# smly/RiichiEnv

Hardware: AMD Instinct MI355X
Metric: env.step()/s (whole node) at 65 536 parallel 4p games; bit-exact MJAI parity (higher is better)
Workload: dtype u8

## Files before the change

riichienv_amd/csrc/rmj_step4.hip.h:

```cpp
namespace RMJ_NS {

#define R4_LIST 16
#define R4_ACT_CAP (KSANMA ? 2 * R4_LIST : R4_LIST)
#define R4_RE_DRAW 1u
#define R4_RE_RESTART 2u
#define R4_RE_PUB 3u
#define R4_RE_YAKU_CLAIMS 4u
#define R4_RE_YAKU_TSUMO 5u
#define R4_RE_WIN_TSUMO 6u
#define R4_RE_WIN_RON 7u
#define R4_RET_ROUND 0x100u
#define STEP_F_ROWS_SHIFT 20
__device__ __forceinline__ uint32_t r4_rows(uint32_t flags) {
    const uint32_t c = (flags >> STEP_F_ROWS_SHIFT) & 3u;
    return c == 0u ? 4u : c;
}
#ifdef RMJ_CUTS
#define R4M(id) do { if (rmj::g_cut == (id)) asm volatile("s_endpgm" ::: "memory"); } while (0)
#define R4BAIL(q, id) do { (q).bail = true; if ((q).r == 0) atomicAdd(&rmj::g_bail_reason[id], 1u); } while (0)
#else
#define R4M(id) do {} while (0)
#ifdef RMJ_CENSUS
#define R4BAIL(q, id) do { (q).bail = true; (q).why = (id); } while (0)
#elif defined(RMJ_TL4)
// ... 253 lines not shown
            const bool ok = live && r4_word_ok(w + (1u << sh3), s, tot);
            W |= (uint64_t)(rballot(ok, rb) & 0x1FFu) << (9 * s);
        }
    }
    const int pairs = __popc(h.a & O9_2 & ~(h.a << 1)) + __popc(h.b & O9_2 & ~(h.b << 1)) + __popc(h.c & O9_2 & ~(h.c << 1)) +
                      __popc(h.d & O7_2 & ~(h.d << 1));
    const uint32_t pres_d = (h.d | (h.d >> 1) | (h.d >> 2)) & O7_1;
    const int kinds = __popc(pres_d) + ((h.a & 7u) != 0u) + ((h.a >> 24) != 0u) + ((h.b & 7u) != 0u) + ((h.b >> 24) != 0u) +
                      ((h.c & 7u) != 0u) + ((h.c >> 24) != 0u);
    if (__ballot(pairs >= 6 || kinds >= 12)) {
        if (pairs >= 6) {
            const uint32_t odd_a = h.a & O9_1, odd_b = h.b & O9_1, odd_c = h.c & O9_1, odd_d = h.d & O7_1;
            const uint32_t four = (h.a & O9_4) | (h.b & O9_4) | (h.c & O9_4) | (h.d & O7_4);
            const int n_odd = __popc(odd_a) + __popc(odd_b) + __popc(odd_c) + __popc(odd_d);
            const int n_two = __popc(h.a & O9_2) + __popc(h.b & O9_2) + __popc(h.c & O9_2) + __popc(h.d & O7_2);
            if (four == 0u && n_odd == 1 && n_two == 6) {
                const int t = odd_a ? (__ffs((int)odd_a) - 1) / 3 : (odd_b ? 9 + (__ffs((int)odd_b) - 1) / 3 : (odd_c ? 18 + (__ffs((int)odd_c) - 1) / 3 : 27 + (__ffs((int)odd_d) - 1) / 3));
                if (ph_cnt(h, t) == 1) W |= 1ull << t;
            }
        }
        if (kinds >= 12) {
            const int t = r < 6 ? (r >> 1) * 9 + (r & 1) * 8 : 27 + (r - 6);
            bool kw = false;
            if (r < 13 && ph_cnt(h, t) < 4) {
                PH x = h;
                ph_add(x, t);
                kw = is_kokushi(x);
            }
            const uint32_t kb = rballot(kw, rb);
            uint64_t kmask = 0ull;
#pragma unroll
            for (int i = 0; i < 13; i++) {
                const int ti = i < 6 ? (i >> 1) * 9 + (i & 1) * 8 : 27 + (i - 6);
                kmask |= (uint64_t)((kb >> i) & 1u) << ti;
            }
            W |= kmask;
        }
    }
    return W;
}

template <bool RICH>
__device__ __forceinline__ void r4_fill_waits13(R4& q, PState* P, int n) {
    uint64_t W = 0ull;
    const R4Shape sp = r4_shape_sorted(q, P, n);
    const int iso = sp.iso, yaochu = sp.yaochu;
    int lb = iso >= 6 ? 4 : (iso == 5 ? 3 : (iso == 4 ? 2 : 0));
    const int len3 = n / 3;
    if (len3 == 4) {
        const int koku = 12 - yaochu;
        lb = koku < lb ? koku : lb;
        if (lb > 2) {
            const int chi = 6 - sp.pairs + (sp.kinds < 7 ? 7 - sp.kinds : 0);
            lb = chi < lb ? chi : lb;
        }
    }
    int sh = lb;
    if (lb < 2) {
        bool far = iso >= 2 && yaochu < 12;
        if (q.gf && !far && !(len3 == 4 && (sp.pairs >= 6 || yaochu >= 12))) {
            const uint32_t gr = r4_group_residues(sp.start, sp.S, n, q.r, q.rb);
            far = gr != 0x01u && gr != 0x20u;
        }
        if (far) {
            sh = 1;
        } else {
            PH h13 = {0, 0, 0, 0};
            {
                uint32_t a = 0, b = 0, c = 0, d = 0;
                if (q.r < n) {
                    const int t = P->hand[q.r] >> 2, su = t_suit(t);
                    const uint32_t one = 1u << (3 * (t - 9 * su));
                    a = su == 0 ? one : 0u; b = su == 1 ? one : 0u; c = su == 2 ? one : 0u; d = su == 3 ? one : 0u;
                }
                a = row_sum16(a); b = row_sum16(b); c = row_sum16(c); d = row_sum16(d);
                const int l15 = q.rb + 15;
                h13.a = (uint32_t)rbc((int)a, l15); h13.b = (uint32_t)rbc((int)b, l15); h13.c = (uint32_t)rbc((int)c, l15); h13.d = (uint32_t)rbc((int)d, l15);
            }
            sh = r4_shanten(q, h13, len3);
            if (sh <= 0) {
                if (!RICH) { R4BAIL(q, 2); return; }
                W = r4_waits_probe(h13.a, h13.b, h13.c, h13.d);
                sh = 0;
            }
        }
    }
    if (q.r == 0) {
        P->waits13 = W;
        P->sh13 = (uint8_t)sh;
        P->flags |= PF_WAITS_VALID;
    }
    wave_sync();
}

template <bool RICH>
__device__ __forceinline__ void r4_fill_waits13_h(R4& q, PState* P, const PH& h13) {
    uint64_t W = 0ull;
    const uint32_t T9 = 1u | (1u << 24);
    const int yaochu = __popc((h13.a | (h13.a >> 1) | (h13.a >> 2)) & T9) + __popc((h13.b | (h13.b >> 1) | (h13.b >> 2)) & T9) +
                       __popc((h13.c | (h13.c >> 1) | (h13.c >> 2)) & T9) + __popc((h13.d | (h13.d >> 1) | (h13.d >> 2)) & O7_1);
    const int iso = r4_isolated(h13);
    int lb = iso >= 6 ? 4 : (iso == 5 ? 3 : (iso == 4 ? 2 : 0));
    const int len3 = ph_total(h13) / 3;
    if (len3 == 4) {
        const int koku = 12 - yaochu;
        lb = koku < lb ? koku : lb;
        if (lb > 2) {
            const int chi = sh_chiitoi(h13, false);
            lb = chi < lb ? chi : lb;
        }
    }
    int sh = lb;
    if (lb < 2) {
        if (iso >= 2 && yaochu < 12) {
            sh = 1;
        } else {
            sh = r4_shanten(q, h13, len3);
            if (sh <= 0) {
                if (!RICH) { R4BAIL(q, 2); return; }
                W = r4_waits_probe(h13.a, h13.b, h13.c, h13.d);
                sh = 0;
            }
        }
    }
    if (q.r == 0) {
        P->waits13 = W;
        P->sh13 = (uint8_t)sh;
        P->flags |= PF_WAITS_VALID;
    }
    wave_sync();
}

__device__ __forceinline__ void r4_accept_riichi(R4& q) {
    GState* G = q.G;
    const int p = G->riichi_pending;
    if (p != 0xFF) {
        q.dirty |= 1u << p;
        if (q.r == 0) {
            G->p[p].score -= 1000;
            G->p[p].score_delta -= 1000;
            G->riichi_sticks += 1;
            G->p[p].flags |= PF_RIICHI_DECLARED | PF_IPPATSU;
            G->riichi_pending = 0xFF;
        }
        wave_sync();
        r4_emit_simple(q, RMJ_EV_REACH_ACCEPTED, (uint32_t)p, 0);
    }
}
__device__ __forceinline__ void r4_check_abortive(R4& q) {
    GState* G = q.G;
    const int p = (q.r >> 2) & 3, m = q.r & 3;
    const PState& P = G->p[p];
    const bool seat_lane = m == 0;
    const int nm = P.n_melds;
    const uint32_t turns_ok = rballot(seat_lane && P.n_discards == 1, q.rb);
    const uint32_t has_melds = rballot(seat_lane && nm != 0, q.rb);
    const uint32_t riichi = rballot(seat_lane && (P.flags & PF_RIICHI_DECLARED), q.rb);
    const uint32_t kan = rballot(m < nm && P.meld_type[m] >= RMJ_MELD_DAIMINKAN, q.rb);
    const uint32_t all_seats = 0x1111u;
    if (!KSANMA && turns_ok == all_seats && has_melds == 0u) {
        const int first = G->p[0].discards[0] >> 2;
        if (first >= 27 && first <= 30) {
            const uint32_t same = rballot(seat_lane && (P.discards[0] >> 2) == first, q.rb);
            if (same == all_seats) R4BAIL(q, 4);
        }
    }
    if (__popc(kan) == 4) {
        const int owner = (__ffs((int)kan) - 1) >> 2;
        if (kan & ~(0xFu << (4 * owner))) R4BAIL(q, 5);
    }
    if (!KSANMA && riichi == all_seats) R4BAIL(q, 6);
}
__device__ __forceinline__ void r4_deal_next(R4& q, int pf) {
    GState* G = q.G;
    const int drawable = G->drawable_count;
    if (drawable == 0) {
        if (q.pause_ok) q.rend = 1u ;
        else { R4BAIL(q, 7); q.cont = 1; }
        return;
    }
    const int live_end = G->live_end;
    const int pid = G->current_player;
    PState* P = &G->p[pid];
    const int hl = P->hand_len;
    if (live_end > G->rinshan_count) {
        q.dirty |= 1u << pid;
        if (q.r == 0) {
            G->is_rinshan = 0;
            G->live_end = (uint8_t)(live_end - 1);
            G->drawable_count = (uint8_t)(drawable - 1);
            if (hl < 14) { P->hand[hl] = (uint8_t)pf; P->hand_len = (uint8_t)(hl + 1); }
            G->drawn_tile = (uint8_t)pf;
            G->needs_tsumo = 0;
            G->phase = RMJ_WAIT_ACT;
            G->active_mask = (uint8_t)(1u << pid);
            P->n_forbidden = 0;
        }
        wave_sync();
        r4_emit_simple(q, RMJ_EV_TSUMO, (uint32_t)pid, (uint32_t)pf);
    } else if (q.r == 0) {
        G->is_rinshan = 0;
    }
}
__device__ __forceinline__ void r4_turn_end(R4& q, int pf) {
    GState* G = q.G;
    r4_accept_riichi(q);
    if (q.tend == 1) r4_check_abortive(q);
    if (q.bail) return;
    const uint32_t tc = G->turn_count + 1u;
    const int pid = G->current_player;
    if (q.r == 0) {
        G->turn_count = tc;
        G->current_player = (uint8_t)(pid + 1 == KNP ? 0 : pid + 1);
    }
    wave_sync();
    r4_deal_next(q, pf);
    if (q.bail) return;
    if (q.r == 0 && tc >= (uint32_t)KNP) G->is_first_turn = 0;
    wave_sync();
}

__device__ __forceinline__ int r4_tile_id(int t34) {
    return KSANMA ? (t34 == 0 ? 0 : (t34 == 8 ? 1 : t34 - 7)) : t34;
}
__device__ __forceinline__ void r4_put(R4& q, int seat, int pos, uint64_t a, int id) {
    if (pos < R4_ACT_CAP) (&q.T->lst[q.row][seat][0])[pos] = a | ((uint64_t)(uint32_t)id << 56);
}

template <bool LOOP>
__device__ __forceinline__ int r4_wall_tile(const R4& q, int idx) {
    const uint8_t* Wg = q.E->wall + (size_t)q.g * RMJ_WALL_STRIDE;
    if (LOOP) {
        const uint32_t w = __hip_atomic_load(reinterpret_cast<const uint32_t*>(Wg) + (idx >> 2), __ATOMIC_RELAXED, __HIP_MEMORY_SCOPE_AGENT);
        return (int)((w >> (8 * (idx & 3))) & 0xFFu);
    }
    return Wg[idx];
}
template <bool LOOP>
__device__ __forceinline__ void r4_flush_kan_dora(R4& q, int extra) {
    GState* G = q.G;
    int pk = (int)G->pending_kan_dora + extra;
    while (__ballot(pk > 0)) {
        if (pk > 0) {
            pk -= 1;
            const int count = G->n_dora;
            const int widx = KSANMA ? 8 + 2 * count : 4 + 2 * count;
            const bool flip = count < 5 && (KSANMA || widx < (int)G->live_end);
            const int t = flip ? r4_wall_tile<LOOP>(q, widx) : 0;
            if (q.r == 0) {
                G->pending_kan_dora = (uint8_t)(pk >= extra ? pk - extra : 0);
                if (flip) { G->dora[count] = (uint8_t)t; G->n_dora = (uint8_t)(count + 1); }
            }
            wave_sync();
            if (flip) r4_emit_simple(q, RMJ_EV_DORA, 0u, (uint32_t)t);
        }
    }
}
template <bool LOOP>
__device__ __forceinline__ void r4_kan_draw(R4& q, int pid, PState* P, bool ankan, uint32_t ev_w0, uint32_t ev_cons, uint32_t ev_n) {
    GState* G = q.G;
    const int r = q.r;
    if (G->drawable_count == 0) { R4BAIL(q, 29); return; }
    if (r < 4) G->p[r].flags &= ~PF_IPPATSU;
    const int rc = G->rinshan_count;
    const int t = r4_wall_tile<LOOP>(q, rc);
    if (r == 0) {
        G->is_first_turn = 0;
        G->rinshan_count = (uint8_t)(rc + 1);
        G->drawable_count -= 1;
        const int h2 = P->hand_len;
        if (h2 < 14) { P->hand[h2] = (uint8_t)t; P->hand_len = (uint8_t)(h2 + 1); }
        G->drawn_tile = (uint8_t)t;
        G->is_rinshan = 1;
    }
    wave_sync();
    if (ev_w0) r4_emit(q, ev_w0, ev_cons, (ev_n << 4) & 0xFFu);
    r4_flush_kan_dora<LOOP>(q, ankan ? 1 : 0);
    if (!ankan && r == 0) G->pending_kan_dora += 1;
    wave_sync();
    r4_emit_simple(q, RMJ_EV_TSUMO, (uint32_t)pid, (uint32_t)t);
    if (r == 0) {
        G->phase = RMJ_WAIT_ACT;
        G->active_mask = (uint8_t)(1u << pid);
    }
    wave_sync();
}
template <bool SETTLE>
__device__ __forceinline__ E4Out r4_seat_eval(uint32_t on, uint32_t seat, uint32_t tile, uint32_t cf, uint32_t honba, bool use_ura, const uint8_t* Wg) {
    const int lane = threadIdx.x & 63, row = lane >> 4, r = lane & 15, rb = lane & 48;
    const GState* G = &g_q4.st[row];
    const PState* P = &G->p[seat & 3u];
    const bool act = on != 0u;
    const int hl = act ? (int)P->hand_len : 0, nm = act ? (int)P->n_melds : 0;
    const int tid = r < hl ? (int)P->hand[r] : 0;
    uint32_t ca = 0, cb = 0, cc = 0, cd = 0;
    if (r < hl) {
        const int t = tid >> 2, su = t_suit(t);
        const uint32_t one = 1u << (3 * (t - 9 * su));
        ca = su == 0 ? one : 0u; cb = su == 1 ? one : 0u; cc = su == 2 ? one : 0u; cd = su == 3 ? one : 0u;
    }
    PH h;
    h.a = e4_rsum(ca, rb); h.b = e4_rsum(cb, rb); h.c = e4_rsum(cc, rb); h.d = e4_rsum(cd, rb);
    int aka = __popc(e4_ballot(r < hl && is_aka(tid), rb));
    uint32_t ma_ = 0, mb_ = 0, mc_ = 0, md_ = 0;
    E4Meld mp;
    {
        const bool mv = r < nm;
        const int m = r & 3;
        const uint32_t type = P->meld_type[m];
        const int nt = type >= RMJ_MELD_DAIMINKAN ? 4 : 3;
        const uint32_t t0 = P->meld_tiles[m][0], t1 = P->meld_tiles[m][1], t2 = P->meld_tiles[m][2], t3 = P->meld_tiles[m][3];
        if (mv) {
#pragma unroll
            for (int k = 0; k < 4; k++) {
                const int t = (int)(k == 0 ? t0 : (k == 1 ? t1 : (k == 2 ? t2 : t3))) >> 2;
                if (k < nt) {
                    const int su = t_suit(t);
                    const uint32_t one = 1u << (3 * (t - 9 * su));
                    ma_ += su == 0 ? one : 0u; mb_ += su == 1 ? one : 0u; mc_ += su == 2 ? one : 0u; md_ += su == 3 ? one : 0u;
                }
            }
        }
        mp = e4_meld_lane(mv, type, nt, t0, t1, t2, t3, (int)((type == RMJ_MELD_CHI ? min(t0, min(t1, t2)) : t0) >> 2), type != RMJ_MELD_CHI,
                          type != RMJ_MELD_ANKAN);
// ... 135 lines not shown
    const PState& S4 = G->p[r & 3];
    const bool other = r < KNP && r != pid;
    const uint32_t qfl = S4.flags;
    const bool holds13 = other && (S4.hand_len + 3 * S4.n_melds == 13);
    const uint64_t W = holds13 ? S4.waits13 : 0ull;
    const uint32_t riichi_m = rballot(r < 4 && (qfl & PF_RIICHI_DECLARED), rb) & 0xFu;
    uint32_t ron_m = 0u;
    if (__ballot(((W >> tt) & 1ull) != 0ull)) {
        const uint64_t dtm = S4.discard_type_mask;
        const bool in_discards = (dtm >> tt) & 1ull;
        const bool in_missed = (qfl & PF_MISSED_DOUJUN) || ((qfl & PF_RIICHI_DECLARED) && (qfl & PF_MISSED_RIICHI));
        const bool furiten = (W & dtm) != 0ull || (qfl & (PF_MISSED_RIICHI | PF_MISSED_DOUJUN));
        ron_m = rballot(other && !in_discards && !in_missed && !furiten && ((W >> tt) & 1ull), rb) & 0xFu;
    }
    if (ron_m && !RICH) { R4BAIL(q, 9); return; }
    if (RICH && (ron_m & ~riichi_m)) {
        if (!RESUME) {
            if (q.pause_ok) q.rend = R4_RE_YAKU_CLAIMS; else R4BAIL(q, 9);
            return;
        }
        const uint32_t ok_m = (ron_m & riichi_m) | (q.yk & ron_m & ~riichi_m), miss_m = (q.yk >> 4) & ron_m & ~riichi_m;
        if (r < 4 && ((miss_m >> r) & 1u)) G->p[r].flags |= PF_MISSED_DOUJUN;
        q.dirty |= miss_m;
        ron_m = ok_m;
        wave_sync();
    }
    w_mine = r < 4 ? W : 0ull;
    const bool can_call = G->drawable_count > 0;
    const bool kuikae = (q.E->rule_bits & RMJ_RULE_KUIKAE_FORBIDDEN) != 0;
    R4M(52);
    int nl0 = (RICH && (ron_m & 1u)) ? 1 : 0, nl1 = (RICH && (ron_m & 2u)) ? 1 : 0, nl2 = (RICH && (ron_m & 4u)) ? 1 : 0, nl3 = (RICH && (ron_m & 8u)) ? 1 : 0;
    auto nl_get = [&](int i) { return i == 0 ? nl0 : (i == 1 ? nl1 : (i == 2 ? nl2 : nl3)); };
    auto nl_set = [&](int i, int v) {
        nl0 = i == 0 ? v : nl0; nl1 = i == 1 ? v : nl1; nl2 = i == 2 ? v : nl2; nl3 = i == 3 ? v : nl3;
    };
#pragma unroll
    for (int k = 1; k < KNP; k++) {
        const int i = pid + k >= KNP ? pid + k - KNP : pid + k;
        const PState* Q = &G->p[i];
        const int hl = Q->hand_len;
        const int ht = r < hl ? (int)Q->hand[r] : 0xFF;
        const uint32_t sm = can_call ? rballot(r < hl && (ht >> 2) == tt, rb) : 0u;
        const int count = __popc(sm);
        if (count < 2 || ((riichi_m >> i) & 1u)) continue;
        const int i0 = __ffs((int)sm) - 1;
        const uint32_t m1 = sm & (sm - 1u);
        const int i1 = __ffs((int)m1) - 1;
        const int i2 = count >= 3 ? __ffs((int)(m1 & (m1 - 1u))) - 1 : 0;
        const uint32_t h0 = (uint32_t)rbc(ht, rb + i0), h1 = (uint32_t)rbc(ht, rb + i1), h2 = (uint32_t)rbc(ht, rb + i2);
        int n = nl_get(i);
        if (r == 0) {
            if (hl >= 3 && (kuikae ? (hl - count) > 0 : (hl - 2) > 0)) {
                r4_put(q, i, n, mk_action(RMJ_PON, tile, 2, h0, h1), KSANMA ? 28 : 41);
                if (count >= 3) {
                    r4_put(q, i, n + 1, mk_action(RMJ_PON, tile, 2, h0, h2), KSANMA ? 28 : 41);
                    r4_put(q, i, n + 2, mk_action(RMJ_PON, tile, 2, h1, h2), KSANMA ? 28 : 41);
                }
            }
        }
        if (hl >= 3 && (kuikae ? (hl - count) > 0 : (hl - 2) > 0)) n += count >= 3 ? 3 : 1;
        if (count >= 3) {
            if (r == 0) r4_put(q, i, n, mk_action(RMJ_DAIMINKAN, tile, 3, h0, h1, h2), (KSANMA ? 29 : 42) + r4_tile_id(tt));
            n += 1;
        }
        nl_set(i, n);
    }
    R4M(53);
    if (!KSANMA && can_call && tt < 27) {
        const int i = (pid + 1) & 3;
        const PState* Q = &G->p[i];
        const int hl = Q->hand_len;
        if (!((riichi_m >> i) & 1u) && hl >= 3) {
            const int ht = r < hl ? (int)Q->hand[r] : 0xFF;
            const int hty = ht >> 2;
            const int r9 = tt % 9;
            const uint32_t m_m2 = rballot(r < hl && hty == tt - 2, rb), m_m1 = rballot(r < hl && hty == tt - 1, rb);
            const uint32_t m_p1 = rballot(r < hl && hty == tt + 1, rb), m_p2 = rballot(r < hl && hty == tt + 2, rb);
            if ((m_m2 && m_m1) || (m_m1 && m_p1) || (m_p1 && m_p2)) {
                const uint32_t m_0 = rballot(r < hl && hty == tt, rb);
                const uint32_t m_p3 = rballot(r < hl && hty == tt + 3, rb), m_m3 = rballot(r < hl && hty == tt - 3, rb);
                const int a = (r >> 2) & 3, b = r & 3;
                int n = nl_get(i);
#pragma unroll
                for (int k = 0; k < 3; k++) {
                    const bool pat_ok = k == 0 ? (r9 >= 2) : (k == 1 ? (r9 >= 1 && r9 <= 7) : (r9 <= 6));
                    const uint32_t ma = k == 0 ? m_m2 : (k == 1 ? m_m1 : m_p1);
                    const uint32_t mbb = k == 0 ? m_m1 : (k == 1 ? m_p1 : m_p2);
                    if (!__ballot(pat_ok && ma != 0u && mbb != 0u)) continue;
                    int forb = __popc(m_0);
                    if (k == 2 && r9 <= 5) forb += __popc(m_p3);
                    if (k == 0 && r9 >= 3) forb += __popc(m_m3);
                    const bool kk_ok = kuikae ? (hl - 2 - forb) > 0 : (hl - 2) > 0;
                    const bool valid = pat_ok && a < __popc(ma) && b < __popc(mbb) && kk_ok;
                    uint32_t x = ma, y = mbb;
                    for (int s = 0; s < a; s++) x &= x - 1u;
                    for (int s = 0; s < b; s++) y &= y - 1u;
                    const int ia = valid ? __ffs((int)x) - 1 : 0, ib = valid ? __ffs((int)y) - 1 : 0;
                    const uint32_t ta = (uint32_t)rbc(ht, rb + ia), tb = (uint32_t)rbc(ht, rb + ib);
                    const uint32_t vb = rballot(valid, rb);
                    if (valid) r4_put(q, i, n + __popc(vb & ((1u << r) - 1u)), mk_action(RMJ_CHI, tile, 2, ta, tb), 40 - k);
                    n += __popc(vb);
                }
                nl_set(i, n);
            }
        }
    }
    R4M(54);
    int n_me = r < 4 ? nl_get(r) : 0;
    if (RICH && ron_m) {
        if (r < 4 && ((ron_m >> r) & 1u)) q.T->lst[q.row][r][0] = mk_action(RMJ_RON, tile, 0) | ((uint64_t)(KSANMA ? 56 : 79) << 56);
        if (r == 0) G->ron_offer_mask = (uint8_t)ron_m;
    }
    if (rballot(r < 4 && n_me + 1 > R4_LIST, rb)) { R4BAIL(q, 10); return; }
    if (r < 4) {
        G->stale_n[r] = (uint8_t)(n_me > 62 ? 62 : n_me);
        if (n_me > 0) {
            q.T->lst[q.row][r][n_me] = mk_action(RMJ_PASS, RMJ_TILE_NONE, 0) | ((uint64_t)(KSANMA ? 58 : 81) << 56);
            n_me += 1;
        }
    }
    nl_mine = r < 4 ? n_me : 0;
    const uint32_t claim_active = rballot(r < 4 && n_me > 0, rb) & 0xFu;
    wave_sync();
    R4M(55);
    if (claim_active) {
        if (r == 0) {
            G->phase = RMJ_WAIT_RESPONSE;
            G->active_mask = (uint8_t)claim_active;
        }
        wave_sync();
    } else {
        q.tend = 1;
    }
}

__device__ __forceinline__ uint32_t r4_tenpai_keep(const R4& q, const PState* P, const PH& full, int hl);
template <bool RICH>
__device__ __forceinline__ void r4_gen_act_legal(R4& q, int& nl_mine) {
    GState* G = q.G;
    const int r = q.r, rb = q.rb;
    const int pid = G->current_player;
    PState* P = &G->p[pid];
    const int hl = P->hand_len, nmelds = P->n_melds;
    const uint32_t pflags = P->flags;
    const bool r_decl = pflags & PF_RIICHI_DECLARED, r_stage = pflags & PF_RIICHI_STAGE;
    const int drawn_tile = G->drawn_tile;
    const bool drawn = drawn_tile != 0xFF;
    const int drawable = G->drawable_count;
    if (hl + 3 * nmelds == 13 || (!RICH && r_stage)) { R4BAIL(q, 11); return; }
    const int ht = r < hl ? (int)P->hand[r] : 0xFF;
    const int hty = ht >> 2;
    int n = 0;
    int d_idx = -1;
    if (drawn && !r_stage) {
        const uint32_t b = rballot(r < hl && ht == drawn_tile, rb);
        const int idx = b ? 31 - __clz((int)b) : -1;
        d_idx = idx;
        const int same_type = __popc(rballot(r < hl && hty == (drawn_tile >> 2), rb));
        if (!(idx >= 0 && same_type <= 4 && (hl - 1) + 3 * nmelds == 13)) { R4BAIL(q, 12); return; }
        if (!(pflags & PF_WAITS_VALID)) {
            const int nx = __builtin_amdgcn_update_dpp(0xFFFF, ht, 0x101 , 0xf, 0xf, false);
            if (idx != hl - 1 || rballot(r < hl - 2 && ht > nx, rb)) r4_fill_waits13_h<RICH>(q, P, r4_hist(q, P, idx));
            else r4_fill_waits13<RICH>(q, P, hl - 1);
            if (q.bail) return;
        }
        if ((P->waits13 >> (drawn_tile >> 2)) & 1ull) {
            const bool concealed = rballot(r < nmelds && P->meld_type[r & 3] != RMJ_MELD_ANKAN, rb) == 0u;
            if (!RICH) { R4BAIL(q, 13); return; }
            bool offer = concealed;
            if (!concealed) {
                if (q.yk_mode == R4_RE_YAKU_TSUMO) offer = (q.yk & 1u) != 0u;
                else if (q.pause_ok) { q.rend = R4_RE_YAKU_TSUMO; return; }
                else { R4BAIL(q, 13); return; }
            }
            if (offer) {
                if (r == 0) r4_put(q, pid, n, mk_action(RMJ_TSUMO, drawn_tile, 0), KSANMA ? 56 : 79);
                n += 1;
            }
        }
    }
    R4M(60);
    const int nforb = P->n_forbidden;
    const bool forb = (nforb > 0 && (P->forbidden[0] >> 2) == hty) || (nforb > 1 && (P->forbidden[1] >> 2) == hty);
    const PH full = r4_hist(q, P, -1);
    if (r_decl) {
        if (drawn) {
            if (r == 0) r4_put(q, pid, n, mk_action(RMJ_DISCARD, drawn_tile, 0), r4_tile_id(drawn_tile >> 2));
            n += 1;
        }
    } else {
        const bool all_closed = rballot(r < nmelds && P->meld_type[r & 3] != RMJ_MELD_ANKAN, rb) == 0u;
        const bool riichi_pre = !r_stage && P->score >= 1000 && (KSANMA ? drawable > 0 : drawable >= 4) && all_closed;
        bool need_tp = r_stage;
        if (riichi_pre) {
            const int sh13 = (drawn && (P->flags & PF_WAITS_VALID)) ? (int)P->sh13 : -1;
            if (sh13 < 2) {
                auto yaochu_kinds = [&]() {
                    const uint32_t T9 = 1u | (1u << 24);
                    return __popc((full.a | (full.a >> 1) | (full.a >> 2)) & T9) + __popc((full.b | (full.b >> 1) | (full.b >> 2)) & T9) +
                           __popc((full.c | (full.c >> 1) | (full.c >> 2)) & T9) + __popc((full.d | (full.d >> 1) | (full.d >> 2)) & O7_1);
                };
                bool may;
                const int nx14 = __builtin_amdgcn_update_dpp(0xFFFF, ht, 0x101 , 0xf, 0xf, false);
                if (q.gf && d_idx == hl - 1 && rballot(r < hl - 2 && ht > nx14, rb) == 0u) {
                    const bool in = r < hl;
                    const int k = in ? r4_key(hty) : 1000;
                    const int kd = rbc(k, rb + hl - 1);
                    const int m = __popc(rballot(r < hl - 1 && k <= kd, rb));
                    const int ks = __builtin_amdgcn_update_dpp(-1000, k, 0x111 , 0xf, 0xf, false);
                    const int k14 = !in ? 1000 : (r < m ? k : (r == m ? kd : ks));
                    const int kp = __builtin_amdgcn_update_dpp(-1000, k14, 0x111 , 0xf, 0xf, false);
                    const bool start = in && k14 - kp > 2;
                    const uint32_t S = rballot(start, rb);
                    const uint32_t gr = r4_group_residues(start, S, hl, r, rb);
                    may = gr == 0x10u || gr == 0x02u || gr == 0x21u;
                    if (!may && hl == 14) {
                        const int kn = __builtin_amdgcn_update_dpp(1000, k14, 0x101 , 0xf, 0xf, false);
                        may = __popc(rballot(in && k14 != kp && k14 == kn, rb)) >= 6 || (__popc(S) >= 12 && yaochu_kinds() >= 12);
                    }
                } else {
                    may = !(r4_isolated(full) >= 3 && yaochu_kinds() < 12);
                }
                if (may) {
                    if (r4_shanten(q, full, hl / 3) <= 0) {
                        if (!RICH) { R4BAIL(q, 14); return; }
                        need_tp = true;
                    }
                }
            }
        }
        uint32_t tp = 0u;
        if (r_stage && G->tp_seat == pid && G->tp_step == G->step_count) {
            tp = G->tp_mask;
            need_tp = false;
        }
        if (RICH && __ballot(need_tp)) {
            if (need_tp) {
                tp = r4_tenpai_keep(q, P, full, hl);
                if (r == 0 && !r_stage) { G->tp_seat = (uint8_t)pid; G->tp_mask = (uint16_t)tp; G->tp_step = G->step_count + 1u; }
            }
        }
        const bool ok = r < hl && !forb && (!r_stage || ((tp >> r) & 1u));
        const uint32_t vb = rballot(ok, rb);
        if (ok) r4_put(q, pid, n + __popc(vb & ((1u << r) - 1u)), mk_action(RMJ_DISCARD, ht, 0), r4_tile_id(hty));
        n += __popc(vb);
        if (riichi_pre && tp != 0u) {
            if (r == 0) r4_put(q, pid, n, mk_action(RMJ_RIICHI, RMJ_TILE_NONE, 0), KSANMA ? 27 : 37);
            n += 1;
        }
    }
    R4M(61);
    if (drawable > 0 && drawn) {
        if (!r_decl && !r_stage) {
            const bool any4 = (((full.a | full.b | full.c) & O9_4) | (full.d & O7_4)) != 0u;
            if (any4) {
                const int next_t = __builtin_amdgcn_update_dpp(0xFFFF, ht, 0x101 , 0xf, 0xf, false);
                if (rballot(r < hl - 2 && ht > next_t, rb)) { R4BAIL(q, 15); return; }
                const int prev_ty = __builtin_amdgcn_update_dpp(-1, hty, 0x111 , 0xf, 0xf, false);
                const bool is4 = r < hl - 1 && hty != prev_ty && ph_cnt(full, hty) == 4;
                const uint32_t ab = rballot(is4, rb);
                if (is4) {
                    const uint32_t lo = (uint32_t)hty * 4u;
                    r4_put(q, pid, n + __popc(ab & ((1u << r) - 1u)), mk_action(RMJ_ANKAN, lo, 4, lo, lo + 1, lo + 2, lo + 3),
                           (KSANMA ? 29 : 42) + r4_tile_id(hty));
                }
                n += __popc(ab);
            }
            const uint32_t pon_lane = rballot(r < nmelds && P->meld_type[r & 3] == RMJ_MELD_PON, rb);
            if (pon_lane) {
                for (int m = 0; m < nmelds; m++) {
                    if (P->meld_type[m] != RMJ_MELD_PON) continue;
                    const int target = P->meld_tiles[m][0] >> 2;
                    const bool hit = r < hl && hty == target;
                    const uint32_t kb = rballot(hit, rb);
                    if (hit)
                        r4_put(q, pid, n + __popc(kb & ((1u << r) - 1u)),
                               mk_kakan(ht, P->meld_tiles[m][0], P->meld_tiles[m][1], P->meld_tiles[m][2]),
                               (KSANMA ? 29 : 42) + r4_tile_id(target));
                    n += __popc(kb);
                }
            }
        } else if (r_decl) {
            if (ph_cnt(full, drawn_tile >> 2) == 4) { R4BAIL(q, 16); return; }
        }
    }
    if (G->is_first_turn && !r_stage && (G->p[0].n_melds | G->p[1].n_melds | G->p[2].n_melds | G->p[3].n_melds) == 0) {
        const bool term = r < hl && is_terminal_tile136(ht);
        const uint32_t lo = row_or16(term && hty < 32 ? 1u << hty : 0u), hi = row_or16(term && hty >= 32 ? 1u << (hty - 32) : 0u);
        const int kinds = __popc((uint32_t)rbc((int)lo, rb + 15)) + __popc((uint32_t)rbc((int)hi, rb + 15));
        if (kinds >= 9) {
            if (r == 0) r4_put(q, pid, n, mk_action(RMJ_KYUSHU, RMJ_TILE_NONE, 0), KSANMA ? 57 : 80);
            n += 1;
        }
    }
    if (KSANMA && drawn && drawable > 0) {
        const bool hit = r < hl && hty == 30;
        const uint32_t kb = rballot(hit, rb);
        if (hit) r4_put(q, pid, n + __popc(kb & ((1u << r) - 1u)), mk_action(RMJ_KITA, ht, 0), 59);
        n += __popc(kb);
    }
    if (n > R4_ACT_CAP) { R4BAIL(q, 17); return; }
    nl_mine = r == pid ? n : 0;
    wave_sync();
}

__device__ __forceinline__ void r4_emit_now(R4& q, bool on, uint32_t w) {
    if (q.E->skip_log) return;
    const uint32_t evc = q.G->ev_count;
    wave_sync();
    if (on) {
        uint32_t* dst = reinterpret_cast<uint32_t*>(q.E->events + (size_t)q.g * (q.E->ring_mask + 1u) + (evc & q.E->ring_mask));
        if (q.r < 8) dst[q.r] = q.r == 7 ? ((w & 0x00FFFFFFu) | ((uint32_t)KNP << 24)) : w;
        if (q.r == 0) q.G->ev_count = evc + 1u;
    }
    wave_sync();
}
#ifdef RMJ_RE_PROF
#define RE_MARK(k) do { const unsigned long long t__ = __builtin_amdgcn_s_memrealtime(); if (lane == 0) atomicAdd(&rmj::g_re_prof[k], t__ - re_t); re_t = t__; } while (0)
#define RE_ROWS(md) do { if ((threadIdx.x & 15u) == 0u) atomicAdd(&rmj::g_re_prof[8 + ((md) & 15u)], 1ull); } while (0)
#define RE_STAMP(t) const unsigned long long t = __builtin_amdgcn_s_memrealtime()
#define RE_ROUND_END_DONE(t) do { if ((threadIdx.x & 63u) == 0u) { const unsigned long long tr = __builtin_amdgcn_s_memrealtime(); atomicAdd(&rmj::g_re_prof[0], tr - t); atomicAdd(&rmj::g_re_prof[1], 1ull); atomicAdd(&rmj::g_re_prof[17], t); atomicAdd(&rmj::g_re_prof[19], tr); } } while (0)
#define RE_PASS2_DONE(t) do { if ((threadIdx.x & 63u) == 0u) { atomicAdd(&rmj::g_re_prof[2], __builtin_amdgcn_s_memrealtime() - t); atomicAdd(&rmj::g_re_prof[3], 1ull); } } while (0)
#else
#define RE_MARK(k) do {} while (0)
#define RE_ROWS(md) do {} while (0)
#define RE_STAMP(t) do {} while (0)
#define RE_ROUND_END_DONE(t) do {} while (0)
#define RE_PASS2_DONE(t) do {} while (0)
#endif
template <bool RICH>
__device__ __noinline__ void r4_round_end(const Env* Ep, uint32_t g0) {
    const int lane = threadIdx.x & 63, row = lane >> 4, r = lane & 15, rb = lane & 48;
#ifdef RMJ_RE_PROF
    unsigned long long re_t = __builtin_amdgcn_s_memrealtime();
    if (lane == 0) atomicAdd(&rmj::g_re_prof[16], re_t);
#endif
    Quad4Shared& sh = g_q4;
    const uint32_t mode = sh.rmode[row];
    CEnv& E = *(CEnv*)uni_ptr(Ep);
    g0 = uni(g0);
    GState* G = &sh.st[row];
    R4 q;
    q.G = G; q.T = &sh.u.t; q.E = &E; q.lane = lane; q.r = r; q.rb = rb; q.row = row; q.g = g0 + (uint32_t)row;
    q.live = mode != 0u; q.bail = false; q.cont = 0; q.rend = mode; q.tend = 0; q.evn = 0; q.dirty = 0xFu; q.pause_ok = false; q.yk = 0u; q.yk_mode = 0u; q.gf = false;
    const bool draw = mode == R4_RE_DRAW, restart = mode == R4_RE_RESTART;
    const bool win_t = mode == R4_RE_WIN_TSUMO, win_r = mode == R4_RE_WIN_RON, win = win_t || win_r;
    bool newround = restart;
    int n_oya = 0, n_rw = 0, n_honba = 0;
    uint32_t n_sticks = 0u;
    const bool seat = r < KNP;
    const int oya = G->oya;
    bool oya_won = false;
    if (RICH && __ballot(win)) {
        const uint8_t* Wg = E.wall + (size_t)q.g * RMJ_WALL_STRIDE;
        const uint32_t rules = E.rule_bits;
        const bool from_discard = G->last_discard_pid != 0xFF;
        const int target = (win_r && from_discard) ? (int)G->last_discard_pid : (int)G->current_player;
        const int win_tile = win_t ? (G->drawn_tile != 0xFF ? (int)G->drawn_tile : 0) : (from_discard ? (int)G->last_discard_tile : 0);
        const uint32_t ron_m = win_r ? (sh.yk[row] & 0xFu) : 0u;
        const uint32_t honba0 = G->honba;
        int32_t total_d = 0;
        bool honba_taken = false, deposit_taken = false;
        for (int dist = 0; dist < KNP; dist++) {
            int w = target + dist;
            w = w >= KNP ? w - KNP : w;
            const bool on = dist == 0 ? win_t : (win_r && ((ron_m >> w) & 1u) != 0u);
            if (!__ballot(on)) continue;
            const PState& Wp = G->p[w & 3];
            const uint32_t wfl = on ? (uint32_t)Wp.flags : 0u;
            const bool riichi = (wfl & PF_RIICHI_DECLARED) != 0u;
            uint32_t cf = (riichi ? CF_RIICHI : 0u) | ((wfl & PF_DOUBLE_RIICHI) ? CF_DOUBLE_RIICHI : 0u) | ((wfl & PF_IPPATSU) ? CF_IPPATSU : 0u);
            const bool last_tile = G->drawable_count == 0 && !G->is_rinshan;
            if (win_t) {
                cf |= CF_TSUMO;
                if (last_tile) cf |= CF_HAITEI;
                if (G->is_rinshan) cf |= CF_RINSHAN;
                const bool no_melds = (G->p[0].n_melds | G->p[1].n_melds | G->p[2].n_melds | G->p[3].n_melds) == 0;
                if (G->is_first_turn && no_melds) cf |= CF_FIRST_TURN;
            } else {
                if (last_tile) cf |= CF_HOUTEI;
                if (G->pending_kan_pid != 0xFF && a_type(G->pending_kan_action) != RMJ_KITA) cf |= CF_CHANKAN;
            }
            const uint32_t hb = honba_taken ? 0u : honba0;
            if (on) honba_taken = true;
            E4Out o = r4_seat_eval<true>(on ? 1u : 0u, (uint32_t)w, (uint32_t)win_tile, cf, hb, riichi, Wg);
            const bool w_oya = w == oya;
            if (o.yakuman && o.han > 13) {
                int cap = 0;
                if (((o.ym >> 47) & 1ull) && !(rules & RMJ_RULE_JUNSEI_CHUUREN_DOUBLE)) cap += 13;
                if (((o.ym >> 48) & 1ull) && !(rules & RMJ_RULE_SUUANKOU_TANKI_DOUBLE)) cap += 13;
                if (((o.ym >> 49) & 1ull) && !(rules & RMJ_RULE_KOKUSHI13_DOUBLE)) cap += 13;
                if (((o.ym >> 50) & 1ull) && !(rules & RMJ_RULE_DAISUUSHII_DOUBLE)) cap += 13;
                if (cap > 0) {
                    const int hh = o.han > cap ? o.han - cap : 0;
                    o.han = hh < 13 ? 13 : hh;
                    const ScoreOut s2 = calc_score((uint32_t)o.han, 0u, w_oya, win_t, hb, (uint32_t)KNP);
                    o.ron = s2.ron; o.tsumo_oya = s2.tsumo_oya; o.tsumo_ko = s2.tsumo_ko;
                }
            }
            const bool won = on && o.is_win;
            int total_val = 0, pao_val = 0, pao_seat = -1;
            if (won && o.yakuman) {
                const uint64_t ids = (0x7FFull << 35) | (0xFull << 47);
                total_val = __popcll(o.ym & ids);
                if (((o.ym >> 47) & 1ull) && (rules & RMJ_RULE_JUNSEI_CHUUREN_DOUBLE)) total_val += 1;
                if (((o.ym >> 48) & 1ull) && (rules & RMJ_RULE_SUUANKOU_TANKI_DOUBLE)) total_val += 1;
                if (((o.ym >> 49) & 1ull) && (rules & RMJ_RULE_KOKUSHI13_DOUBLE)) total_val += 1;
                const int v50 = (rules & RMJ_RULE_DAISUUSHII_DOUBLE) ? 2 : 1;
                if (((o.ym >> 50) & 1ull) && v50 == 2) total_val += 1;
                if (((o.ym >> 37) & 1ull) && Wp.pao37 != 0xFF) { pao_val += 1; pao_seat = Wp.pao37; }
                if (((o.ym >> 50) & 1ull) && Wp.pao50 != 0xFF) { pao_val += v50; pao_seat = Wp.pao50; }
            }
            const int32_t sticks = (won && !deposit_taken) ? (int32_t)(G->riichi_sticks * 1000u) : 0;
            int32_t d = 0;
            {
                if (won && win_t && r < KNP && r != w) {
                    if (pao_val > 0) {
                        const int32_t unit = w_oya ? (KNP - 1) * 16000 : 16000 + (KNP - 2) * 8000;
                        const int32_t honba_total = (int32_t)hb * (KNP - 1) * 100;
                        if (rules & RMJ_RULE_PAO_LIABILITY_ONLY) {
                            const int32_t non = total_val - pao_val;
                            if (non > 0) d -= (w_oya || r == oya) ? non * 16000 : non * 8000;
                            if (r == pao_seat) d -= pao_val * unit + honba_total;
                        } else if (r == pao_seat) {
                            d -= total_val * unit + honba_total;
                        }
                    } else {
                        d = -(int32_t)(w_oya ? o.tsumo_ko : (r == oya ? o.tsumo_oya : o.tsumo_ko));
                    }
                }
                const int32_t tw = -(int32_t)e4_rsum((uint32_t)d, rb);
                if (won && win_t && r == w) d = tw + sticks;
            }
            if (won && win_r) {
                const int32_t score = (int32_t)o.ron;
                int payer = target;
// ... 1609 lines not shown
```

Before: 2.149 billion.

## Skip full hand histogram and abortive-draw ballots when sorted-run shortcuts suffice

The abortive-draw check now does a cheap wave-wide test for whether any of the four-winds, four-riichi or four-kan conditions could apply, and returns early otherwise. Action generation builds the full hand histogram (r4_hist) only when shanten, tenpai or kan detection actually needs it. In the common case where the drawn tile extends an already sorted 13-tile run, ankan detection, the yaochu count and the four-of-a-kind bail test are done with lane-wise DPP and ballot operations instead. This removes histogram construction and several ballots from the per-step hot path, but adds more branches and more complex lane-count logic that must stay bit-exact.

```diff
diff --git a/riichienv_amd/csrc/rmj_step4.hip.h b/riichienv_amd/csrc/rmj_step4.hip.h
--- a/riichienv_amd/csrc/rmj_step4.hip.h
+++ b/riichienv_amd/csrc/rmj_step4.hip.h
@@ -429,24 +429,33 @@
     const int p = (q.r >> 2) & 3, m = q.r & 3;
     const PState& P = G->p[p];
     const bool seat_lane = m == 0;
-    const int nm = P.n_melds;
-    const uint32_t turns_ok = rballot(seat_lane && P.n_discards == 1, q.rb);
-    const uint32_t has_melds = rballot(seat_lane && nm != 0, q.rb);
-    const uint32_t riichi = rballot(seat_lane && (P.flags & PF_RIICHI_DECLARED), q.rb);
-    const uint32_t kan = rballot(m < nm && P.meld_type[m] >= RMJ_MELD_DAIMINKAN, q.rb);
     const uint32_t all_seats = 0x1111u;
-    if (!KSANMA && turns_ok == all_seats && has_melds == 0u) {
+    const PState& D = G->p[G->current_player];
+    const bool meld_lane = m < (int)P.n_melds;
+    const uint32_t melds = rballot(meld_lane, q.rb);
+    const bool winds_q = !KSANMA && D.n_discards == 1 && (melds & all_seats) == 0u;
+    const bool riichi_q = !KSANMA && (D.flags & PF_RIICHI_DECLARED);
+    const bool kans_q = __popc(melds) >= 4;
+    if (!__ballot(winds_q || riichi_q || kans_q)) return;
+    if (winds_q) {
+        const uint32_t turns_ok = rballot(seat_lane && P.n_discards == 1, q.rb);
         const int first = G->p[0].discards[0] >> 2;
-        if (first >= 27 && first <= 30) {
+        if (turns_ok == all_seats && first >= 27 && first <= 30) {
             const uint32_t same = rballot(seat_lane && (P.discards[0] >> 2) == first, q.rb);
             if (same == all_seats) R4BAIL(q, 4);
         }
     }
-    if (__popc(kan) == 4) {
-        const int owner = (__ffs((int)kan) - 1) >> 2;
-        if (kan & ~(0xFu << (4 * owner))) R4BAIL(q, 5);
-    }
-    if (!KSANMA && riichi == all_seats) R4BAIL(q, 6);
+    if (kans_q) {
+        const uint32_t kan = rballot(meld_lane && P.meld_type[m] >= RMJ_MELD_DAIMINKAN, q.rb);
+        if (__popc(kan) == 4) {
+            const int owner = (__ffs((int)kan) - 1) >> 2;
+            if (kan & ~(0xFu << (4 * owner))) R4BAIL(q, 5);
+        }
+    }
+    if (riichi_q) {
+        const uint32_t riichi = rballot(seat_lane && (P.flags & PF_RIICHI_DECLARED), q.rb);
+        if (riichi == all_seats) R4BAIL(q, 6);
+    }
 }
 __device__ __forceinline__ void r4_deal_next(R4& q, int pf) {
     GState* G = q.G;
@@ -888,15 +897,16 @@
     const int hty = ht >> 2;
     int n = 0;
     int d_idx = -1;
+    const int nx = __builtin_amdgcn_update_dpp(0xFFFF, ht, 0x101 , 0xf, 0xf, false);
+    const bool sorted13 = rballot(r < hl - 2 && ht > nx, rb) == 0u;
+    const int same_type = drawn ? __popc(rballot(r < hl && hty == (drawn_tile >> 2), rb)) : 0;
     if (drawn && !r_stage) {
         const uint32_t b = rballot(r < hl && ht == drawn_tile, rb);
         const int idx = b ? 31 - __clz((int)b) : -1;
         d_idx = idx;
-        const int same_type = __popc(rballot(r < hl && hty == (drawn_tile >> 2), rb));
         if (!(idx >= 0 && same_type <= 4 && (hl - 1) + 3 * nmelds == 13)) { R4BAIL(q, 12); return; }
         if (!(pflags & PF_WAITS_VALID)) {
-            const int nx = __builtin_amdgcn_update_dpp(0xFFFF, ht, 0x101 , 0xf, 0xf, false);
-            if (idx != hl - 1 || rballot(r < hl - 2 && ht > nx, rb)) r4_fill_waits13_h<RICH>(q, P, r4_hist(q, P, idx));
+            if (idx != hl - 1 || !sorted13) r4_fill_waits13_h<RICH>(q, P, r4_hist(q, P, idx));
             else r4_fill_waits13<RICH>(q, P, hl - 1);
             if (q.bail) return;
         }
@@ -918,27 +928,21 @@
     R4M(60);
     const int nforb = P->n_forbidden;
     const bool forb = (nforb > 0 && (P->forbidden[0] >> 2) == hty) || (nforb > 1 && (P->forbidden[1] >> 2) == hty);
-    const PH full = r4_hist(q, P, -1);
-    if (r_decl) {
-        if (drawn) {
-            if (r == 0) r4_put(q, pid, n, mk_action(RMJ_DISCARD, drawn_tile, 0), r4_tile_id(drawn_tile >> 2));
-            n += 1;
-        }
-    } else {
+    const bool run14 = d_idx == hl - 1 && sorted13;
+    bool riichi_pre = false, need_tp = false, may = false, may_hist = false;
+    uint32_t tp = 0u;
+    if (!r_decl) {
         const bool all_closed = rballot(r < nmelds && P->meld_type[r & 3] != RMJ_MELD_ANKAN, rb) == 0u;
-        const bool riichi_pre = !r_stage && P->score >= 1000 && (KSANMA ? drawable > 0 : drawable >= 4) && all_closed;
-        bool need_tp = r_stage;
+        riichi_pre = !r_stage && P->score >= 1000 && (KSANMA ? drawable > 0 : drawable >= 4) && all_closed;
+        need_tp = r_stage;
+        if (r_stage && G->tp_seat == pid && G->tp_step == G->step_count) {
+            tp = G->tp_mask;
+            need_tp = false;
+        }
         if (riichi_pre) {
             const int sh13 = (drawn && (P->flags & PF_WAITS_VALID)) ? (int)P->sh13 : -1;
             if (sh13 < 2) {
-                auto yaochu_kinds = [&]() {
-                    const uint32_t T9 = 1u | (1u << 24);
-                    return __popc((full.a | (full.a >> 1) | (full.a >> 2)) & T9) + __popc((full.b | (full.b >> 1) | (full.b >> 2)) & T9) +
-                           __popc((full.c | (full.c >> 1) | (full.c >> 2)) & T9) + __popc((full.d | (full.d >> 1) | (full.d >> 2)) & O7_1);
-                };
-                bool may;
-                const int nx14 = __builtin_amdgcn_update_dpp(0xFFFF, ht, 0x101 , 0xf, 0xf, false);
-                if (q.gf && d_idx == hl - 1 && rballot(r < hl - 2 && ht > nx14, rb) == 0u) {
+                if (q.gf && run14) {
                     const bool in = r < hl;
                     const int k = in ? r4_key(hty) : 1000;
                     const int kd = rbc(k, rb + hl - 1);
@@ -952,23 +956,36 @@
                     may = gr == 0x10u || gr == 0x02u || gr == 0x21u;
                     if (!may && hl == 14) {
                         const int kn = __builtin_amdgcn_update_dpp(1000, k14, 0x101 , 0xf, 0xf, false);
-                        may = __popc(rballot(in && k14 != kp && k14 == kn, rb)) >= 6 || (__popc(S) >= 12 && yaochu_kinds() >= 12);
+                        const bool first = in && k14 != kp;
+                        may = __popc(rballot(first && k14 == kn, rb)) >= 6 ||
+                              (__popc(S) >= 12 && __popc(rballot(first && (k14 >= 48 || (k14 & 7) == 0), rb)) >= 12);
                     }
                 } else {
-                    may = !(r4_isolated(full) >= 3 && yaochu_kinds() < 12);
-                }
-                if (may) {
-                    if (r4_shanten(q, full, hl / 3) <= 0) {
-                        if (!RICH) { R4BAIL(q, 14); return; }
-                        need_tp = true;
-                    }
-                }
-            }
-        }
-        uint32_t tp = 0u;
-        if (r_stage && G->tp_seat == pid && G->tp_step == G->step_count) {
-            tp = G->tp_mask;
-            need_tp = false;
+                    may_hist = true;
+                }
+            }
+        }
+    }
+    const bool need_full = may || may_hist || need_tp || (drawable > 0 && drawn && !r_decl && !r_stage && !run14);
+    PH full = {0u, 0u, 0u, 0u};
+    if (__ballot(need_full)) full = r4_hist(q, P, -1);
+    if (r_decl) {
+        if (drawn) {
+            if (r == 0) r4_put(q, pid, n, mk_action(RMJ_DISCARD, drawn_tile, 0), r4_tile_id(drawn_tile >> 2));
+            n += 1;
+        }
+    } else {
+        if (may_hist) {
+            const uint32_t T9 = 1u | (1u << 24);
+            const int yaochu = __popc((full.a | (full.a >> 1) | (full.a >> 2)) & T9) + __popc((full.b | (full.b >> 1) | (full.b >> 2)) & T9) +
+                               __popc((full.c | (full.c >> 1) | (full.c >> 2)) & T9) + __popc((full.d | (full.d >> 1) | (full.d >> 2)) & O7_1);
+            may = !(r4_isolated(full) >= 3 && yaochu < 12);
+        }
+        if (may) {
+            if (r4_shanten(q, full, hl / 3) <= 0) {
+                if (!RICH) { R4BAIL(q, 14); return; }
+                need_tp = true;
+            }
         }
         if (RICH && __ballot(need_tp)) {
             if (need_tp) {
@@ -988,12 +1005,25 @@
     R4M(61);
     if (drawable > 0 && drawn) {
         if (!r_decl && !r_stage) {
-            const bool any4 = (((full.a | full.b | full.c) & O9_4) | (full.d & O7_4)) != 0u;
+            bool any4;
+            if (run14) {
+                const int ty3 = __builtin_amdgcn_update_dpp(-1, hty, 0x103 , 0xf, 0xf, false);
+                any4 = same_type >= 4 || rballot(r + 3 < hl - 1 && hty == ty3, rb) != 0u;
+            } else {
+                any4 = (((full.a | full.b | full.c) & O9_4) | (full.d & O7_4)) != 0u;
+            }
             if (any4) {
-                const int next_t = __builtin_amdgcn_update_dpp(0xFFFF, ht, 0x101 , 0xf, 0xf, false);
-                if (rballot(r < hl - 2 && ht > next_t, rb)) { R4BAIL(q, 15); return; }
+                if (!sorted13) { R4BAIL(q, 15); return; }
                 const int prev_ty = __builtin_amdgcn_update_dpp(-1, hty, 0x111 , 0xf, 0xf, false);
-                const bool is4 = r < hl - 1 && hty != prev_ty && ph_cnt(full, hty) == 4;
+                const bool starter = r < hl - 1 && hty != prev_ty;
+                int cnt;
+                if (run14) {
+                    const uint32_t rest = rballot(starter, rb) >> (r + 1);
+                    cnt = (rest ? __ffs((int)rest) : hl - 1 - r) + (hty == (drawn_tile >> 2) ? 1 : 0);
+                } else {
+                    cnt = ph_cnt(full, hty);
+                }
+                const bool is4 = starter && cnt == 4;
                 const uint32_t ab = rballot(is4, rb);
                 if (is4) {
                     const uint32_t lo = (uint32_t)hty * 4u;
@@ -1017,7 +1047,7 @@
                 }
             }
         } else if (r_decl) {
-            if (ph_cnt(full, drawn_tile >> 2) == 4) { R4BAIL(q, 16); return; }
+            if (same_type == 4) { R4BAIL(q, 16); return; }
         }
     }
     if (G->is_first_turn && !r_stage && (G->p[0].n_melds | G->p[1].n_melds | G->p[2].n_melds | G->p[3].n_melds) == 0) {
```

Measured after the change: 2.176 billion (median of 6 runs). 1.01x the previous value.
